# pityka/lamp

Hardware: AMD Instinct MI355X
Metric: training-step samples/sec (higher is better)
Workload: dtype bf16; 1 GPU; example-cifar100 Cnn.resnet(100) training step (fwd+backprop+AdamW), synthetic CIFAR batch; per_gpu_batch=2048, global_batch=2048, parallelism=single, optimizer=AdamW lr 1e-3 wd 0 beta2 0.95 mixedPrecision

## Files before the change

### lamp_amd/csrc/core/switches.h

```cpp
#pragma once
#include <cstdint>

namespace lamp {

constexpr int64_t SW_NO_CLAMP = INT64_MIN;

#define LAMP_SWITCHES_ONCE(X)                                                                                                             \
                                                        \
  X(conv_sibling, "LAMP_CONV_SIBLING", BOOL, 1, 0, "a residual block's 3x3 and its sibling 1x1 of the same input as one forward launch") \
  X(conv_chain, "LAMP_CONV_CHAIN", BOOL, 1, 0, "a convolution directly in front of a residual block and the block's 3x3 + 1x1 as one forward call (0: two)") \
  X(fuse_bn_pair, "LAMP_FUSE_BN_PAIR", BOOL, 1, 0, "relu(bn(right) + bn(left)) at a block's end as one op (0: the chain)")                \
  X(fuse_pool_logsoftmax, "LAMP_FUSE_POOL_LOGSOFTMAX", BOOL, 1, 0, "average pool -> flatten -> log-softmax tail as one node")             \
  X(fuse_block_tail, "LAMP_FUSE_BLOCK_TAIL", BOOL, 1, 0, "the last residual block and the pooled log-softmax tail as one node")          \
  X(fuse_bn_conv, "LAMP_FUSE_BN_CONV", BOOL, 1, 0, "batch norm -> relu -> convolution: the convolution applies the norm while staging")  \
  X(fuse_loss_accumulate, "LAMP_FUSE_LOSS_ACCUMULATE", BOOL, 1, 0, "acc += n * loss inside the NLL loss kernel")                          \
  X(fuse_loss_backward, "LAMP_FUSE_LOSS_BACKWARD", BOOL, 1, 0, "the NLL loss backward goes straight to the pooled log-softmax node's input in one launch")                      \
  X(fuse_loss_tail, "LAMP_FUSE_LOSS_TAIL", BOOL, 1, 0, "the loss launch also writes the pooled log-softmax's input gradient per plane")  \
  X(conv_dgrad_accumulate, "LAMP_CONV_DGRAD_ACCUMULATE", BOOL, 1, 0, "a convolution's input gradient adds into the existing one in its epilogue") \
  X(conv_dgrad_pair, "LAMP_CONV_DGRAD_PAIR", BOOL, 1, 0, "input gradients of a block's 3x3 and sibling 1x1 from one launch")             \
  X(conv_wgrad_pair, "LAMP_CONV_WGRAD_PAIR", BOOL, 1, 0, "weight gradients of a block's 3x3 and sibling 1x1 from one launch")            \
  X(conv_bwd_pair, "LAMP_CONV_BWD_PAIR", BOOL, 1, 0, "a block's paired input gradient and its two weight gradients from one call (0: the two pair calls)") \
  X(linear_bias_fused, "LAMP_LINEAR_BIAS_FUSED", BOOL, 1, 0, "a linear layer's bias in the GEMM epilogue (0: mm then add)")               \
  X(mult_add_fused, "LAMP_MULT_ADD_FUSED", BOOL, 1, 0, "x * scale + residual in one pass (0: mult then add)")                             \
  X(attention_as_written_for_cuda, "LAMP_ATTENTION_AS_WRITTEN_FOR_CUDA", BOOL, 0, 0, "multi-head attention as the reference's op chain instead of the fused kernels") \
  X(recurrent_fused, "LAMP_RECURRENT_FUSED", BOOL, 1, 0, "RNN / GRU / LSTM as one node per sequence with fused cell kernels (0: the fold over time steps)") \
  X(fuse_qkv, "LAMP_FUSE_QKV", BOOL, 1, 0, "self-attention's three projections as one product (0: three)")                                \
  X(host_stream_side, "LAMP_HOST_STREAM_SIDE", BOOL, 0, 0, "batch streams gather on a side stream instead of the consumer's")             \
                                                                           \
  X(pinned_cache_mb, "LAMP_PINNED_CACHE_MB", INT, 2048, 0, "upper bound of the cache of freed pinned host buffers, MiB")                  \
  X(pinned_gather_wgs, "LAMP_PINNED_GATHER_WGS", INT, 48, 1, "workgroups of a gather that reads pinned host memory")                      \
                                                                                                    \
  X(flash_attention, "LAMP_FLASH_ATTENTION", BOOL, 1, 0, "the flash attention kernels, forward and backward")                             \
  X(small_attention, "LAMP_SMALL_ATTENTION", BOOL, 1, 0, "the short-sequence attention kernels")                                          \
  X(knn_fused, "LAMP_KNN_FUSED", BOOL, 1, 0, "the fused distance + top-k nearest-neighbour kernel")                                       \
  X(knn_split, "LAMP_KNN_SPLIT", INT, -1, SW_NO_CLAMP, "f16-plane k-NN filter: 0 off, 1 where it pays, 2 forced; negative: the mode set through the API") \
  X(knn_split_planes, "LAMP_KNN_SPLIT_PLANES", INT, 0, SW_NO_CLAMP, "f16 planes per coordinate of that filter: 3, anything else 2")      \
  X(umap_pairs2, "LAMP_UMAP_PAIRS2", BOOL, 1, 0, "the UMAP loss's two-dimensional pair kernel")                                            \
                                                                                                             \
  X(gemm_shape_tags, "LAMP_GEMM_SHAPE_TAGS", BOOL, 0, 0, "profiling aid: one kernel-timer class per GEMM shape and layout")               \
  X(gemm_splitk, "LAMP_GEMM_SPLITK", BOOL, 1, 0, "split-K for products with few output tiles (bf16 and f32 / f64)")                       \
  X(gemm_tail_split, "LAMP_GEMM_TAIL_SPLIT", BOOL, 1, 0, "an almost empty last round of 256 x 256 tiles becomes a second, split-K product") \
  X(gemm_fp_split_wgs, "LAMP_GEMM_FP_SPLIT_WGS", INT, 512, 1, "workgroups an f32 / f64 split-K product aims at")                          \
                                                                                              \
  X(bn_fused_bwd, "LAMP_BN_FUSED_BWD", BOOL, 1, 0, "one-pass batch-norm backward (workgroups exchange their sums) where no mode is set through the API") \
  X(bn_fused_fp, "LAMP_BN_FUSED_FP", BOOL, 1, 0, "... its f32 / f64 form")                                                               \
  X(bn_fused_np_mask, "LAMP_BN_FUSED_NP_MASK", INT, 24, SW_NO_CLAMP, "bit mask of packets per thread (1 .. 16) at which the one-pass form runs") \
  X(bn_fused_per_cu, "LAMP_BN_FUSED_PER_CU", INT, 1, 1, "workgroups per CU the one-pass form aims at first")                              \
  X(bn_fused_small_bytes, "LAMP_BN_FUSED_SMALL_BYTES", INT, (4 << 20) + 1, SW_NO_CLAMP, "bf16 activations below this many bytes take the one-pass form whatever the mask") \
                          \
  X(conv_small2, "LAMP_CONV_SMALL2", BOOL, 1, 0, "the small-map direct convolution kernels (second generation)")                          \
  X(conv_small2_wgrad, "LAMP_CONV_SMALL2_WGRAD", BOOL, 1, 0, "... their weight gradient")                                                 \
  X(igemm_f32, "LAMP_IGEMM_F32", BOOL, 1, 0, "implicit-GEMM convolution for f32")                                                          \
  X(igemm_f64, "LAMP_IGEMM_F64", BOOL, 1, 0, "implicit-GEMM convolution for f64")                                                          \
  X(conv_bn_stats, "LAMP_CONV_BN_STATS", BOOL, 1, 0, "forward convolutions hand per-image batch-norm statistics of their output on")     \
  X(ncv_bn_stats, "LAMP_NCV_BN_STATS", BOOL, 1, 0, "... the narrow kernels' alone (needs LAMP_CONV_BN_STATS on as well)")                 \
  X(ncv_dgrad_parity, "LAMP_NCV_DGRAD_PARITY", BOOL, 1, 0, "narrow stride-2 pair input gradient: super-tiles by row parity (0: the plain form)") \
  X(pack_cache, "LAMP_PACK_CACHE", BOOL, 1, 0, "packed filter images are cached per parameter and storage version (all four packing backends: core/pack_cache.h)") \
  X(pack_after_step, "LAMP_PACK_AFTER_STEP", BOOL, 1, 0, "the optimiser repacks every cached filter image of all four backends in place (0: lazily at first use)") \
                                                    \
  X(ig_small_d, "LAMP_IG_SMALL_D", BOOL, 1, 0, "the eight-image kernel for at most 64 output channels too")                               \
  X(ig_w8, "LAMP_IG_W8", BOOL, 1, 0, "two-image 128-row kernel: eight waves per image pair at one workgroup per CU or fewer (0: four)")  \
  X(ig_one_image, "LAMP_IG_ONE_IMAGE", BOOL, 1, 0, "... one image per workgroup at one image per CU or fewer (0: pairs)")                 \
  X(ig_bwd_pair, "LAMP_IG_BWD_PAIR", BOOL, 1, 0, "a wide block's short-K entry pair: input gradient and both weight gradients from one eight-image launch (0: the two pair calls)") \
  X(ig_fwd_pair, "LAMP_IG_FWD_PAIR", BOOL, 1, 0, "a wide block's short-K entry pair, forward: the barrier-free eight-image kernel with both filters resident in LDS (0: the eight-image kernel's sibling form)") \
                                                                                                 \
  X(wgrad_group, "LAMP_WGRAD_GROUP", BOOL, 1, 0, "two layers' eight-wave weight gradients parked and launched as one (0: every layer at once)") \
  X(wgrad_min_ips, "LAMP_WGRAD_MIN_IPS", INT, 0, 2, "fewest images per weight-gradient workgroup; unset (0): 2 up to 512 images, 8 above") \
  X(wg8h_dma, "LAMP_WG8H_DMA", BOOL, 1, 0, "eight-wave weight-gradient kernel: dY tiles by LDS-DMA (0: through registers, the bitwise reference of the DMA's hand-counted waits)") \
  X(defer_wgrad_reduce, "LAMP_DEFER_WGRAD_REDUCE", BOOL, 1, 0, "weight-gradient partial sums are reduced in batches, deferred until someone reads them")

#define LAMP_SWITCHES_PER_CALL(X)                                                                                                         \
  X(ig_variant, "LAMP_IG_VARIANT", LETTER, 0, 0, "bf16 implicit GEMM kernel form: b two-image 128-row, d eight-image at any batch; unset or any other letter: by geometry") \
  X(ig_ktail, "LAMP_IG_KTAIL", BOOL, 1, 0, "a 3x3's 1 .. 8 channels beyond the last whole K chunk from their own packed image (0: the padded chunk)") \
  X(knn_split_dbg, "LAMP_KNN_SPLIT_DBG", INT, 0, SW_NO_CLAMP, "3: the k-NN filter's kernel counts visits, candidates and selection cycles per wave and prints them")

using SwType_BOOL = bool;
using SwType_INT = int64_t;
using SwType_LETTER = char;
#define LAMP_SWITCH_MEMBER(member, name, kind, dflt, lo, doc) SwType_##kind member;
struct Switches { LAMP_SWITCHES_ONCE(LAMP_SWITCH_MEMBER) };
struct SwitchesNow { LAMP_SWITCHES_PER_CALL(LAMP_SWITCH_MEMBER) };
#undef LAMP_SWITCH_MEMBER

const Switches& sw();
SwitchesNow sw_now();

}
```

### lamp_amd/csrc/kernels/norm.hip

```cpp
#include "device_utils.h"
#include <atomic>
#include <map>
#include <mutex>
#include <type_traits>
#include "../core/strided.h"
#include "../core/switches.h"

namespace lamp {

template <class A> struct Welford {
  A n, mean, m2;
};
template <class A> __device__ __forceinline__ void wf_add(Welford<A>& w, A x) {
  w.n += A(1);
  A d = x - w.mean;
  w.mean += d / w.n;
  w.m2 += d * (x - w.mean);
}
template <class A> __device__ __forceinline__ Welford<A> wf_merge(const Welford<A>& a, const Welford<A>& b) {
  Welford<A> r;
  r.n = a.n + b.n;
  if (r.n == A(0)) { r.mean = 0; r.m2 = 0; return r; }
  A d = b.mean - a.mean;
  A f = b.n / r.n;
// ... 102 lines not shown
  if (c >= C) return;
  mean[c] = running_mean ? running_mean[c] : store_as<T>(A(0));
  const A v = running_var ? load_as<A>(running_var[c]) : A(1);
  invstd[c] = store_as<T>((A)(A(1) / (A)sqrt((double)(v + (A)eps))));
}
template <class A> __device__ __forceinline__ A bn_affine(A x, A mu, A scale, A bb);
template <> __device__ __forceinline__ float bn_affine<float>(float x, float mu, float scale, float bb) { return __builtin_fmaf(x - mu, scale, bb); }
template <> __device__ __forceinline__ double bn_affine<double>(double x, double mu, double scale, double bb) { return __builtin_fma(x - mu, scale, bb); }
template <class T>
__global__ __launch_bounds__(256) void bn_apply_kernel(const T* __restrict__ x, T* __restrict__ y, const T* __restrict__ mean,
                                                       const T* __restrict__ invstd, const T* __restrict__ w, const T* __restrict__ b,
                                                       int64_t total, int64_t C, int64_t HW, int vec, int relu) {
  using A = acc_t<T>;
  constexpr int W = 16 / sizeof(T);
  if (vec) {
    const int64_t vpp = HW / W, nv = total / W;
    for (int64_t i = blockIdx.x * (int64_t)blockDim.x + threadIdx.x; i < nv; i += (int64_t)gridDim.x * blockDim.x) {
      const int64_t c = (i / vpp) % C;
      const A scale = load_as<A>(invstd[c]) * (w ? load_as<A>(w[c]) : A(1));
      const A mu = load_as<A>(mean[c]);
      const A bb = b ? load_as<A>(b[c]) : A(0);
      Vec<T, W> pk = *reinterpret_cast<const Vec<T, W>*>(x + i * W);
#pragma unroll
      for (int k = 0; k < W; k++) {
        T v = store_as<T>(bn_affine<A>(load_as<A>(pk.v[k]), mu, scale, bb));
        if (relu && load_as<A>(v) < A(0)) v = store_as<T>(A(0));
        pk.v[k] = v;
      }
      *reinterpret_cast<Vec<T, W>*>(y + i * W) = pk;
    }
    return;
  }
  for (int64_t i = blockIdx.x * (int64_t)blockDim.x + threadIdx.x; i < total; i += (int64_t)gridDim.x * blockDim.x) {
    const int64_t c = (i / HW) % C;
    const A scale = load_as<A>(invstd[c]) * (w ? load_as<A>(w[c]) : A(1));
    const A bb = b ? load_as<A>(b[c]) : A(0);
    T v = store_as<T>(bn_affine<A>(load_as<A>(x[i]), load_as<A>(mean[c]), scale, bb));
    if (relu && load_as<A>(v) < A(0)) v = store_as<T>(A(0));
    y[i] = v;
  }
}

template <class T>
__device__ __forceinline__ void bn_merge_channel(const acc_t<T>* __restrict__ partial, int nsplit, int64_t c, int64_t C, int slice, T* __restrict__ save_mean,
                                                 T* __restrict__ save_invstd, T* running_mean, T* running_var, double momentum, double eps,
                                                 acc_t<T>* stat, acc_t<T> (*wpart)[3]) {
  using A = acc_t<T>;
  const int np = nsplit < 0 ? -nsplit : nsplit;
  if (nsplit < 0) {
    const A* pc = partial + (int64_t)c * np * 3;
    const A shift = pc[1];
    A s1 = 0, s2 = 0, sm = 0;
    for (int s = threadIdx.x; s < np; s += blockDim.x) { const A d = pc[s * 3 + 1] - shift; s1 += d; s2 += d * d; sm += pc[s * 3 + 2]; }
    s1 = wave_sum(s1); s2 = wave_sum(s2); sm = wave_sum(sm);
    if ((threadIdx.x & 63) == 0) { wpart[threadIdx.x >> 6][0] = s1; wpart[threadIdx.x >> 6][1] = s2; wpart[threadIdx.x >> 6][2] = sm; }
    __syncthreads();
  }
  if (threadIdx.x < 64) {
    const int lane = threadIdx.x;
    Welford<A> r{0, 0, 0};
    if (nsplit < 0) {
      A s1 = 0, s2 = 0, sm = 0;
      for (int k = 0; k < (int)(blockDim.x >> 6); k++) { s1 += wpart[k][0]; s2 += wpart[k][1]; sm += wpart[k][2]; }
      const A n0 = partial[(int64_t)c * np * 3], shift = partial[(int64_t)c * np * 3 + 1];
      r.n = n0 * (A)np;
      r.mean = shift + s1 / (A)np;
      r.m2 = sm + n0 * (s2 - s1 * s1 / (A)np);
    } else {
      for (int s = lane; s < np; s += 64) {
        const A* p = partial + ((int64_t)s * C + c) * 3;
        r = wf_merge(r, Welford<A>{p[0], p[1], p[2]});
      }
      r = wf_wave(r);
    }
    if (lane == 0) {
      const A var_biased = r.m2 / r.n;
      const A invstd = A(1) / (A)sqrt((double)(var_biased + (A)eps));
      const T m_t = store_as<T>(r.mean), is_t = store_as<T>(invstd);
      stat[0] = load_as<A>(m_t);
      stat[1] = load_as<A>(is_t);
      if (slice == 0) {
        save_mean[c] = m_t;
        save_invstd[c] = is_t;
        if (running_mean) running_mean[c] = store_as<T>((A)((A)momentum * r.mean + (A)(1 - momentum) * load_as<A>(running_mean[c])));
        if (running_var) {
          const A unbiased = r.m2 / (r.n - A(1));
          running_var[c] = store_as<T>((A)((A)momentum * unbiased + (A)(1 - momentum) * load_as<A>(running_var[c])));
        }
      }
    }
  }
  __syncthreads();
}
template <class T>
__global__ __launch_bounds__(256) void bn_affine_table_kernel(const acc_t<T>* __restrict__ partial, int nsplit, T* __restrict__ save_mean, T* __restrict__ save_invstd,
                                                              T* running_mean, T* running_var, double momentum, double eps, const T* __restrict__ w,
                                                              const T* __restrict__ b, int64_t C, float4* __restrict__ affine) {
  using A = acc_t<T>;
  __shared__ A stat[2];
  __shared__ A wpart[4][3];
  const int64_t c = blockIdx.x;
  bn_merge_channel<T>(partial, nsplit, c, C, 0, save_mean, save_invstd, running_mean, running_var, momentum, eps, stat, wpart);
  if (threadIdx.x == 0) affine[c] = make_float4((float)stat[0], (float)(stat[1] * (w ? load_as<A>(w[c]) : A(1))), b ? (float)load_as<A>(b[c]) : 0.f, 0.f);
}
template <class T>
__global__ __launch_bounds__(256) void bn_affine_from_saved_kernel(const T* __restrict__ mean, const T* __restrict__ invstd, const T* __restrict__ w,
                                                                   const T* __restrict__ b, int64_t C, float4* __restrict__ affine) {
  using A = acc_t<T>;
  const int64_t c = blockIdx.x * (int64_t)blockDim.x + threadIdx.x;
  if (c < C) affine[c] = make_float4((float)load_as<A>(mean[c]), (float)(load_as<A>(invstd[c]) * (w ? load_as<A>(w[c]) : A(1))), b ? (float)load_as<A>(b[c]) : 0.f, 0.f);
}
template <class T> struct BnSecond {
  const T* x; const acc_t<T>* partial; int nsplit; T* save_mean; T* save_invstd; T* running_mean; T* running_var; double momentum, eps; const T* w; const T* b;
};

template <class T>
__global__ __launch_bounds__(256) void bn_apply2_kernel(const T* __restrict__ x, T* __restrict__ y, const acc_t<T>* __restrict__ partial, int nsplit,
                                                        T* __restrict__ save_mean, T* __restrict__ save_invstd, T* running_mean, T* running_var,
                                                        double momentum, double eps, const T* __restrict__ w, const T* __restrict__ b, int64_t N,
                                                        int64_t C, int64_t HW, int nblk, int vec, int relu, const T* __restrict__ addend,
                                                        BnSecond<T> second, T* __restrict__ pooled = nullptr) {
  using A = acc_t<T>;
  constexpr int W = 16 / sizeof(T);
  __shared__ A stat[2], stat2[2];
  __shared__ A wpart[4][3];
  const int64_t c = blockIdx.x;
  const int slice = blockIdx.y;
  bn_merge_channel<T>(partial, nsplit, c, C, slice, save_mean, save_invstd, running_mean, running_var, momentum, eps, stat, wpart);
  if (second.x)
    bn_merge_channel<T>(second.partial, second.nsplit, c, C, slice, second.save_mean, second.save_invstd, second.running_mean, second.running_var,
                        second.momentum, second.eps, stat2, wpart);
  const A mu = stat[0];
  const A scale = stat[1] * (w ? load_as<A>(w[c]) : A(1));
  const A bb = b ? load_as<A>(b[c]) : A(0);
  const A mu2 = second.x ? stat2[0] : A(0);
  const A scale2 = second.x ? stat2[1] * (second.w ? load_as<A>(second.w[c]) : A(1)) : A(0);
  const A bb2 = (second.x && second.b) ? load_as<A>(second.b[c]) : A(0);
  const T* __restrict__ adsrc = second.x ? second.x : addend;
  if (vec) {
    const int64_t vpp = HW / W, total = N * vpp;
    for (int64_t i = (int64_t)slice * blockDim.x + threadIdx.x; i < total; i += (int64_t)nblk * blockDim.x) {
      const int64_t n = i / vpp, v = i - n * vpp;
      const int64_t base = (n * C + c) * HW + v * W;
      Vec<T, W> pk, ad;
      { const uint4 t = nt_load16(reinterpret_cast<const uint4*>(x + base)); pk = *reinterpret_cast<const Vec<T, W>*>(&t); }
      if (adsrc) { const uint4 t = nt_load16(reinterpret_cast<const uint4*>(adsrc + base)); ad = *reinterpret_cast<const Vec<T, W>*>(&t); }
#pragma unroll
      for (int k = 0; k < W; k++) {
        T o = store_as<T>(bn_affine<A>(load_as<A>(pk.v[k]), mu, scale, bb));
        if (adsrc) {
          T a = ad.v[k];
          if (second.x) a = store_as<T>(bn_affine<A>(load_as<A>(a), mu2, scale2, bb2));
          o = store_as<T>((A)(load_as<A>(o) + load_as<A>(a)));
        }
        if (relu && load_as<A>(o) < A(0)) o = store_as<T>(A(0));
        pk.v[k] = o;
      }
      if (pooled) {
        A sum = 0;
#pragma unroll
        for (int k = 0; k < W; k++) sum += load_as<A>(pk.v[k]);
        for (int off = (int)vpp >> 1; off > 0; off >>= 1) sum += __shfl_xor(sum, off, 64);
        if (v == 0) pooled[n * C + c] = store_as<T>((A)(sum / (A)HW));
      } else *reinterpret_cast<Vec<T, W>*>(y + base) = pk;
    }
  } else {
    const int64_t total = N * HW;
    for (int64_t i = (int64_t)slice * blockDim.x + threadIdx.x; i < total; i += (int64_t)nblk * blockDim.x) {
      const int64_t n = i / HW, v = i - n * HW;
      const int64_t base = (n * C + c) * HW + v;
      T o = store_as<T>(bn_affine<A>(load_as<A>(x[base]), mu, scale, bb));
      if (adsrc) {
        T a = adsrc[base];
        if (second.x) a = store_as<T>(bn_affine<A>(load_as<A>(a), mu2, scale2, bb2));
        o = store_as<T>((A)(load_as<A>(o) + load_as<A>(a)));
      }
      if (relu && load_as<A>(o) < A(0)) o = store_as<T>(A(0));
      y[base] = o;
    }
  }
}

template <class T>
__global__ __launch_bounds__(256) void bn_bwd_reduce_kernel(const T* __restrict__ dy, const T* __restrict__ x, const T* __restrict__ mean,
                                                            acc_t<T>* __restrict__ partial, int64_t N, int64_t C, int64_t HW, int nsplit, int vec,
                                                            int relu, const T* __restrict__ invstd, const T* __restrict__ w, const T* __restrict__ b,
                                                            const T* __restrict__ addend) {
  using A = acc_t<T>;
  constexpr int W = 16 / sizeof(T);
  __shared__ A sm[2][4];
  const int64_t c = blockIdx.x;
  const int split = blockIdx.y;
  const A mu = load_as<A>(mean[c]);
  const A scale = relu ? load_as<A>(invstd[c]) * (w ? load_as<A>(w[c]) : A(1)) : A(0);
  const A bb = (relu && b) ? load_as<A>(b[c]) : A(0);
  A s1 = 0, s2 = 0;
  if (vec) {
    const int64_t vpp = HW / W, total = N * vpp;
    for (int64_t i = (int64_t)split * blockDim.x + threadIdx.x; i < total; i += (int64_t)nsplit * blockDim.x) {
      const int64_t n = i / vpp, v = i - n * vpp;
      const int64_t base = (n * C + c) * HW + v * W;
      const Vec<T, W> g = *reinterpret_cast<const Vec<T, W>*>(dy + base);
      const Vec<T, W> xv = *reinterpret_cast<const Vec<T, W>*>(x + base);
      Vec<T, W> ad;
      if (addend) ad = *reinterpret_cast<const Vec<T, W>*>(addend + base);
#pragma unroll
      for (int k = 0; k < W; k++) {
        A gg = load_as<A>(g.v[k]);
        const A xx = load_as<A>(xv.v[k]);
        if (relu) {
          T pre = store_as<T>(bn_affine<A>(xx, mu, scale, bb));
          if (addend) pre = store_as<T>((A)(load_as<A>(pre) + load_as<A>(ad.v[k])));
          if (load_as<A>(pre) < A(0)) gg = A(0);
        }
        s1 += gg; s2 += gg * (xx - mu);
      }
    }
  } else {
    const int64_t total = N * HW;
    for (int64_t i = (int64_t)split * blockDim.x + threadIdx.x; i < total; i += (int64_t)nsplit * blockDim.x) {
      const int64_t n = i / HW, v = i - n * HW;
      const int64_t base = (n * C + c) * HW + v;
      A gg = load_as<A>(dy[base]);
      const A xx = load_as<A>(x[base]);
      if (relu) {
        T pre = store_as<T>(bn_affine<A>(xx, mu, scale, bb));
        if (addend) pre = store_as<T>((A)(load_as<A>(pre) + load_as<A>(addend[base])));
        if (load_as<A>(pre) < A(0)) gg = A(0);
      }
      s1 += gg; s2 += gg * (xx - mu);
    }
  }
  s1 = wave_sum(s1); s2 = wave_sum(s2);
  const int lane = threadIdx.x & 63, wid = threadIdx.x >> 6;
  if (lane == 0) { sm[0][wid] = s1; sm[1][wid] = s2; }
  __syncthreads();
  if (threadIdx.x == 0) {
    A a = 0, bsum = 0;
    for (int k = 0; k < (int)(blockDim.x >> 6); k++) { a += sm[0][k]; bsum += sm[1][k]; }
    partial[((int64_t)split * C + c) * 2] = a;
    partial[((int64_t)split * C + c) * 2 + 1] = bsum;
  }
}
template <class T>
__global__ __launch_bounds__(256) void bn_bwd_reduce_col_kernel(const T* __restrict__ dy, const T* __restrict__ x, const T* __restrict__ mean,
                                                                acc_t<T>* __restrict__ partial, int64_t N, int64_t C, int64_t HW, int nsplit) {
  using A = acc_t<T>;
  const int64_t c = blockIdx.x * (int64_t)blockDim.x + threadIdx.x;
  if (c >= C) return;
  const int split = blockIdx.y;
  const A mu = load_as<A>(mean[c]);
  A s1 = 0, s2 = 0;
  for (int64_t n = split; n < N; n += nsplit) {
    const int64_t base = (n * C + c) * HW;
    for (int64_t i = 0; i < HW; i++) {
      const A g = load_as<A>(dy[base + i]);
      s1 += g;
      s2 += g * (load_as<A>(x[base + i]) - mu);
    }
  }
  partial[((int64_t)split * C + c) * 2] = s1;
// ... 679 lines not shown
#undef BN_FUSED_K
}
struct BnPlaneGrad { const bf16_t* p = nullptr; int sn = 0, sc = 0; };
template <class T>
static bool bn_bwd_fused_launch(const Tensor* gc, const Tensor* xc, const Tensor* mean_t, const Tensor* invstd_t, const Tensor* weight, const Tensor* bias,
                                Tensor* dw, Tensor* db, Tensor* dx, Tensor* dadd, const Tensor* addc, const BnGeom& g, int relu, hipStream_t st,
                                const BnDualHost* dualh = nullptr, BnPlaneGrad gplanes = BnPlaneGrad()) {
  constexpr bool BF16 = std::is_same<T, bf16_t>::value;
  constexpr int W = 16 / (int)sizeof(T);
  if (!bn_fused_gate(xc->device(), !BF16) || g.HW % W != 0) return false;
  const int64_t packets = g.N * (g.HW / W);
  if (packets <= 0 || packets >= (int64_t)1 << 30 || xc->numel() / W >= (int64_t)1 << 31) return false;
  if (addc && !relu) return false;
  const bool planes = gplanes.p != nullptr;
  if (planes && !(dualh && g.HW == 64 && gplanes.sn == 1 && g.N % 8 == 0 && gplanes.sc % 8 == 0 && ((uintptr_t)gplanes.p & 15) == 0)) return false;
  const int cus = num_cus();
  const int np_mask = (int)sw().bn_fused_np_mask;
  auto resident = [&](const void* k) { return std::min<int64_t>(BN_FUSED_SLOTS, (int64_t)cus * std::max(1, kernel_occupancy(k, 512, 0))); };
  const void* kfn = nullptr;
  int64_t S = 0, chunk = g.C;
  if constexpr (BF16) {
    if (g.C > BN_FUSED_MAXC) return false;
    const bool any_size = dualh || xc->numel() * 2 < sw().bn_fused_small_bytes;
    for (int wgs = (int)sw().bn_fused_per_cu; wgs >= 1 && !kfn; wgs--) {
      const BnFusedSlices sl = bn_fused_slices(packets, g.C, cus, wgs);
      if (!any_size && !(np_mask & sl.NP)) continue;
      const void* k = bn_fused_kernel_for<T>(sl.NP, relu, addc, dualh, planes);
      if (g.C * sl.s <= resident(k)) { kfn = k; S = sl.s; }
    }
    if (!kfn) return false;
  } else {
    const BnFusedSlices sl = bn_fused_slices(packets, g.C, cus, 1);
    if (!(np_mask & sl.NP)) return false;
    kfn = bn_fused_kernel_for<T>(sl.NP, relu, addc, false, false);
    const int64_t r = resident(kfn);
    if (sl.s > r) return false;
    S = sl.s;
    chunk = std::min<int64_t>(std::min<int64_t>(g.C, r / S), BN_FUSED_MAXC);
  }
  BnFusedSync sync = bn_fused_sync_state(xc->device(), st);
  if (!sync.depart) return false;
  const double passes = (dx ? 3.0 : 2.0) + (addc ? 1.0 : 0.0) + (dadd ? 1.0 : 0.0) - (planes ? 1.0 : 0.0);
  KernelTimer kt("bn_bwd_fused", 0, passes * (double)xc->numel() * sizeof(T), st);
  auto in = [](const Tensor* t) { return t ? t->ptr<T>() : (const T*)nullptr; };
  auto out = [](Tensor* t) { return t ? t->ptr<T>() : (T*)nullptr; };
  const T* dyp = in(gc); const T* xp = in(xc); const T* mp = in(mean_t); const T* ip = in(invstd_t); const T* wp = in(weight); const T* bp = in(bias);
  const T* adp = in(addc);
  T* dwp = out(dw); T* dbp = out(db); T* dxp = out(dx); T* dap = out(dadd);
  BnFusedDual<T> dual{};
  int a_sc = 0;
  if constexpr (BF16) {
    if (planes) { dyp = gplanes.p; a_sc = gplanes.sc; }
    if (dualh) dual = BnFusedDual<T>{in(dualh->mean2), in(dualh->invstd2), in(dualh->w2), in(dualh->b2), out(dualh->dw2), out(dualh->db2)};
  }
  int64_t a_N = g.N; int a_C = (int)g.C, a_HW = (int)g.HW, a_S = (int)S;
  double inv_m = 1.0 / (double)(g.N * g.HW);
  int a_vshift = bn_fused_vshift(g.HW / W);
  int* awp = device_assert_word(xc->device());
  for (int64_t c0 = 0; c0 < g.C; c0 += chunk) {
    int a_c0 = (int)c0;
    const int64_t nc = std::min<int64_t>(chunk, g.C - c0);
    void* args[] = {(void*)&dyp, (void*)&xp, (void*)&mp, (void*)&ip, (void*)&wp, (void*)&bp, (void*)&sync.slots, (void*)&sync.slots2, (void*)&sync.depart, (void*)&dwp,
                    (void*)&dbp, (void*)&dxp, (void*)&a_N, (void*)&a_C, (void*)&a_HW, (void*)&a_S, (void*)&inv_m, (void*)&adp, (void*)&dap, (void*)&a_vshift, (void*)&awp,
                    (void*)&a_c0, (void*)&dual, (void*)&a_sc};
    HIP_CHECK(hipLaunchKernel(kfn, dim3((unsigned)(nc * S)), dim3(512), args, 0, st));
  }
  return true;
}
static BnPlaneGrad plane_broadcast_base(const Tensor* g) {
  BnPlaneGrad r;
  if (!g || g->dtype != kBF16 || g->ndim != 4 || !g->is_device()) return r;
  if (g->sizes[2] * g->sizes[3] <= 1 || g->strides[2] != 0 || g->strides[3] != 0) return r;
  const int64_t sn = g->sizes[0] > 1 ? g->strides[0] : 0, sc = g->sizes[1] > 1 ? g->strides[1] : 0;
  if (sn < 0 || sc < 0 || sn >= ((int64_t)1 << 24) || sc >= ((int64_t)1 << 24) || (g->sizes[0] - 1) * sn + (g->sizes[1] - 1) * sc >= ((int64_t)1 << 31)) return r;
  r.p = g->ptr<bf16_t>(); r.sn = (int)sn; r.sc = (int)sc;
  return r;
}
static void check_cvec(const Tensor* t, int64_t C, int dtype, const char* what) {
  if (!t) return;
  check_device_tensor(t, what);
  LAMP_CHECK(t->numel() == C && t->dtype == dtype && t->is_contiguous(), what << " must be a contiguous [" << C << "] tensor of the input dtype, got " << t->describe());
}

}

using namespace lamp;

extern "C" {

int lamp_bn_backward_mode(int mode) {
  LAMP_API_BEGIN
  LAMP_CHECK(mode >= -1 && mode <= 2, "lamp_bn_backward_mode: mode must be -1, 0, 1 or 2");
  g_bn_bwd_mode.store(mode, std::memory_order_relaxed);
  LAMP_API_END
}

struct BnSecondArgs {
  const lamp_tensor* x; const lamp_tensor* weight; const lamp_tensor* bias; lamp_tensor* running_mean; lamp_tensor* running_var; double momentum, eps;
  lamp_tensor* save_mean = nullptr; lamp_tensor* save_invstd = nullptr;
};
static int bn_forward_impl(lamp_tensor* out3[3], const lamp_tensor* x, const lamp_tensor* weight, const lamp_tensor* bias,
                           lamp_tensor* running_mean, lamp_tensor* running_var, int training, double momentum, double eps, int relu,
                           const lamp_tensor* addend = nullptr, BnSecondArgs* second = nullptr, bool table_only = false, bool* pooled = nullptr) {
  LAMP_API_BEGIN
  check_device_tensor(x, "input");
  BnGeom g = bn_geom(x);
  const bool want_pooled = pooled && *pooled;
  if (pooled) *pooled = false;
  LAMP_CHECK(!table_only || (training && !addend && !second && x->dtype != kF64), "the batch norm table exists in training mode, as an f32 table for f32 / f16 / bf16 inputs");
  Hold addc, x2c, mean2, invstd2;
  if (second) {
    check_device_tensor(second->x, "second input");
    LAMP_CHECK(!addend && relu && training && g.HW >= 64, "the two-batch-norm residual tail exists in training mode for maps of at least 64 elements");
    LAMP_CHECK(second->x->shape() == x->shape() && second->x->dtype == x->dtype, "second input " << second->x->describe() << " does not match input " << x->describe());
    check_cvec(second->weight, g.C, x->dtype, "second weight"); check_cvec(second->bias, g.C, x->dtype, "second bias");
    check_cvec(second->running_mean, g.C, x->dtype, "second running_mean"); check_cvec(second->running_var, g.C, x->dtype, "second running_var");
    x2c = Hold(contiguous(second->x));
    int64_t cs2[1] = {g.C};
    mean2 = Hold(new_tensor(cs2, 1, x->dtype, x->device())); invstd2 = Hold(new_tensor(cs2, 1, x->dtype, x->device()));
  }
  if (addend) {
    check_device_tensor(addend, "addend");
    LAMP_CHECK(relu && training && g.HW >= 64, "the fused batch-norm-add-relu exists in training mode for maps of at least 64 elements");
    LAMP_CHECK(addend->shape() == x->shape() && addend->dtype == x->dtype, "addend " << addend->describe() << " does not match input " << x->describe());
    addc = Hold(contiguous(addend));
  }
  check_cvec(weight, g.C, x->dtype, "weight"); check_cvec(bias, g.C, x->dtype, "bias");
  check_cvec(running_mean, g.C, x->dtype, "running_mean"); check_cvec(running_var, g.C, x->dtype, "running_var");
  Hold xc(contiguous(x));
  int64_t cs[1] = {g.C}, ts[2] = {g.C, 4};
  Hold y(table_only ? new_tensor(ts, 2, kF32, x->device()) : new_like(xc.get()));
  Hold pooled_t;
  Hold mean(new_tensor(cs, 1, x->dtype, x->device())), invstd(new_tensor(cs, 1, x->dtype, x->device()));
  hipStream_t st = current_stream(x->device());
  const int64_t total = x->numel();
  LAMP_DISPATCH_FLOAT(x->dtype, T, {
    using A = acc_t<T>;
    const int vec = (g.HW % (16 / sizeof(T)) == 0) && (((uintptr_t)xc->raw() | (uintptr_t)y->raw() | (uintptr_t)(x2c.get() ? x2c->raw() : nullptr)) & 15) == 0;
    float4* table = table_only ? reinterpret_cast<float4*>(y->raw()) : nullptr;
    if (training) {
      LAMP_CHECK(g.N * g.HW > 0, "batch norm over an empty batch");
      const bool col = g.HW < 64;
      const int64_t blocks = col ? (g.C + 255) / 256 : g.C;
      const int nsplit = pick_split(blocks, g.N);
      int npart = nsplit;
      Hold partial;
      if (!col && std::is_same<A, float>::value) partial = Hold(conv_stats_lookup(xc.get(), g.C, &npart));
      const bool have_stats = partial.get() != nullptr;
      if (!have_stats) {
        npart = nsplit;
        int64_t ps[1] = {(int64_t)nsplit * g.C * 3};
        partial = Hold(new_tensor(ps, 1, acc_dtype<A>(), x->device()));
      }
      T* rm = running_mean ? running_mean->ptr<T>() : (T*)nullptr;
      T* rv = running_var ? running_var->ptr<T>() : (T*)nullptr;
      const T* wp = weight ? weight->ptr<T>() : (const T*)nullptr;
      const T* bp = bias ? bias->ptr<T>() : (const T*)nullptr;
      if (!have_stats) {
        KernelTimer kt("bn_fwd_stats", 0, (double)total * sizeof(T), st);
        if (col) hipLaunchKernelGGL((bn_stats_col_kernel<T>), dim3((unsigned)blocks, nsplit), dim3(256), 0, st, static_cast<const Tensor*>(xc.get())->ptr<T>(), partial->ptr<A>(), g.N, g.C, g.HW, nsplit);
        else hipLaunchKernelGGL((bn_stats_kernel<T>), dim3((unsigned)g.C, nsplit), dim3(256), 0, st, static_cast<const Tensor*>(xc.get())->ptr<T>(), partial->ptr<A>(), g.N, g.C, g.HW, nsplit, vec);
        LAMP_LAUNCH_CHECK();
      }
      BnSecond<T> sec{};
      Hold partial2;
      if (second) {
        LAMP_CHECK(!col && total > 0, "the two-batch-norm residual tail needs maps of at least 64 elements");
        int npart2 = nsplit;
        if (std::is_same<A, float>::value) partial2 = Hold(conv_stats_lookup(x2c.get(), g.C, &npart2));
        const bool have2 = partial2.get() != nullptr;
        if (!have2) {
          npart2 = nsplit;
          int64_t ps[1] = {(int64_t)nsplit * g.C * 3};
          partial2 = Hold(new_tensor(ps, 1, acc_dtype<A>(), x->device()));
          KernelTimer kt("bn_fwd_stats", 0, (double)total * sizeof(T), st);
          hipLaunchKernelGGL((bn_stats_kernel<T>), dim3((unsigned)g.C, nsplit), dim3(256), 0, st, static_cast<const Tensor*>(x2c.get())->ptr<T>(), partial2->ptr<A>(), g.N, g.C, g.HW, nsplit, vec);
          LAMP_LAUNCH_CHECK();
        }
        sec.x = static_cast<const Tensor*>(x2c.get())->ptr<T>();
        sec.partial = static_cast<const Tensor*>(partial2.get())->ptr<A>(); sec.nsplit = have2 ? -npart2 : npart2;
        sec.save_mean = mean2->ptr<T>(); sec.save_invstd = invstd2->ptr<T>();
        sec.running_mean = second->running_mean ? second->running_mean->ptr<T>() : (T*)nullptr;
        sec.running_var = second->running_var ? second->running_var->ptr<T>() : (T*)nullptr;
        sec.momentum = second->momentum; sec.eps = second->eps;
        sec.w = second->weight ? second->weight->ptr<T>() : (const T*)nullptr; sec.b = second->bias ? second->bias->ptr<T>() : (const T*)nullptr;
      }
      if (table_only && !col) {
        hipLaunchKernelGGL((bn_affine_table_kernel<T>), dim3((unsigned)g.C), dim3(256), 0, st, static_cast<const Tensor*>(partial.get())->ptr<A>(),
                           have_stats ? -npart : npart, mean->ptr<T>(), invstd->ptr<T>(), rm, rv, momentum, eps, wp, bp, g.C, table);
        LAMP_LAUNCH_CHECK();
      } else if (!col && total > 0) {
        const int vec2 = (vec && (!addc.get() || ((uintptr_t)addc->data() & 15) == 0)) ? 1 : 0;
        const int64_t vpp = g.HW / (int64_t)(16 / sizeof(T));
        T* poolp = nullptr;
        if (want_pooled && second && vec2 && vpp >= 1 && vpp <= 64 && (vpp & (vpp - 1)) == 0) {
          int64_t ps[2] = {g.N, g.C};
          pooled_t = Hold(new_tensor(ps, 2, x->dtype, x->device()));
          poolp = pooled_t->ptr<T>();
          *pooled = true;
        }
        KernelTimer kt("bn_fwd_apply", 0, ((second ? 3.0 : addc.get() ? 3.0 : 2.0) - (poolp ? 1.0 : 0.0)) * (double)total * sizeof(T), st);
        hipLaunchKernelGGL((bn_apply2_kernel<T>), dim3((unsigned)g.C, nsplit), dim3(256), 0, st, static_cast<const Tensor*>(xc.get())->ptr<T>(), y->ptr<T>(),
                           static_cast<const Tensor*>(partial.get())->ptr<A>(), have_stats ? -npart : npart,
                           mean->ptr<T>(), invstd->ptr<T>(), rm, rv, momentum, eps, wp, bp, g.N, g.C, g.HW, nsplit,
                           vec2, relu, addc.get() ? addc->ptr<T>() : (const T*)nullptr, sec, poolp);
        LAMP_LAUNCH_CHECK();
      } else {
        hipLaunchKernelGGL((bn_finalize_kernel<T>), dim3((unsigned)((g.C * 64 + 255) / 256)), dim3(256), 0, st, partial->ptr<A>(), g.C, nsplit,
                           mean->ptr<T>(), invstd->ptr<T>(), rm, rv, momentum, eps);
        LAMP_LAUNCH_CHECK();
        if (table_only) {
          hipLaunchKernelGGL((bn_affine_from_saved_kernel<T>), dim3((unsigned)((g.C + 255) / 256)), dim3(256), 0, st, mean->ptr<T>(), invstd->ptr<T>(), wp, bp, g.C, table);
          LAMP_LAUNCH_CHECK();
        } else if (total > 0) {
          KernelTimer kt("bn_fwd_apply", 0, 2.0 * (double)total * sizeof(T), st);
          hipLaunchKernelGGL((bn_apply_kernel<T>), dim3(grid_for(total, 256)), dim3(256), 0, st, xc->ptr<T>(), y->ptr<T>(), mean->ptr<T>(), invstd->ptr<T>(),
                             wp, bp, total, g.C, g.HW, vec, relu);
          LAMP_LAUNCH_CHECK();
        }
      }
    } else {
      hipLaunchKernelGGL((bn_eval_stats_kernel<T>), dim3((unsigned)((g.C + 255) / 256)), dim3(256), 0, st,
                         running_mean ? running_mean->ptr<T>() : (const T*)nullptr, running_var ? running_var->ptr<T>() : (const T*)nullptr,
                         mean->ptr<T>(), invstd->ptr<T>(), g.C, eps);
      LAMP_LAUNCH_CHECK();
      if (total > 0) {
        KernelTimer kt("bn_fwd_apply", 0, 2.0 * (double)total * sizeof(T), st);
        hipLaunchKernelGGL((bn_apply_kernel<T>), dim3(grid_for(total, 256)), dim3(256), 0, st, xc->ptr<T>(), y->ptr<T>(), mean->ptr<T>(),
                           invstd->ptr<T>(), weight ? weight->ptr<T>() : (const T*)nullptr, bias ? bias->ptr<T>() : (const T*)nullptr, total,
                           g.C, g.HW, vec, relu);
        LAMP_LAUNCH_CHECK();
      }
    }
  });
  if (!training) {
  }
  out3[0] = pooled_t.get() ? pooled_t.take() : y.take(); out3[1] = mean.take(); out3[2] = invstd.take();
  if (second) { second->save_mean = mean2.take(); second->save_invstd = invstd2.take(); }
  LAMP_API_END
}
int lamp_native_batch_norm(lamp_tensor* out3[3], const lamp_tensor* x, const lamp_tensor* weight, const lamp_tensor* bias,
                           lamp_tensor* running_mean, lamp_tensor* running_var, int training, double momentum, double eps) {
  return bn_forward_impl(out3, x, weight, bias, running_mean, running_var, training, momentum, eps, 0);
}
int lamp_native_batch_norm_relu(lamp_tensor* out3[3], const lamp_tensor* x, const lamp_tensor* weight, const lamp_tensor* bias,
                                lamp_tensor* running_mean, lamp_tensor* running_var, int training, double momentum, double eps) {
  return bn_forward_impl(out3, x, weight, bias, running_mean, running_var, training, momentum, eps, 1);
}

int lamp_batch_norm_affine(lamp_tensor* out3[3], const lamp_tensor* x, const lamp_tensor* weight, const lamp_tensor* bias, lamp_tensor* running_mean,
                           lamp_tensor* running_var, double momentum, double eps) {
  return bn_forward_impl(out3, x, weight, bias, running_mean, running_var, 1, momentum, eps, 1, nullptr, nullptr, true);
}

static int bn_backward_impl(lamp_tensor* out3[3], const lamp_tensor* grad_out, const lamp_tensor* x, const lamp_tensor* weight,
                            const lamp_tensor* bias, const lamp_tensor* running_mean, const lamp_tensor* running_var,
                            const lamp_tensor* save_mean, const lamp_tensor* save_invstd, int training, double eps, const uint8_t mask[3],
                            int relu, const lamp_tensor* addend = nullptr, lamp_tensor** daddend_out = nullptr) {
  LAMP_API_BEGIN
  check_device_tensor(x, "input"); check_device_tensor(grad_out, "grad_out");
  LAMP_CHECK(grad_out->shape() == x->shape() && grad_out->dtype == x->dtype, "grad_out " << grad_out->describe() << " does not match input " << x->describe());
  BnGeom g = bn_geom(x);
  check_cvec(weight, g.C, x->dtype, "weight");
  if (relu) {
    check_cvec(bias, g.C, x->dtype, "bias");
    LAMP_CHECK(g.HW >= 64, "the fused batch-norm-relu backward exists for maps of at least 64 elements, got " << x->describe());
  }
  Hold xc(contiguous(x)), gc(contiguous(grad_out));
  Hold addc, dadd;
  if (addend) {
    check_device_tensor(addend, "addend");
    LAMP_CHECK(relu && training, "the fused batch-norm-add-relu backward exists in training mode");
    LAMP_CHECK(addend->shape() == x->shape() && addend->dtype == x->dtype, "addend " << addend->describe() << " does not match input " << x->describe());
    addc = Hold(contiguous(addend));
    if (daddend_out) dadd = Hold(new_like(xc.get()));
  }
  hipStream_t st = current_stream(x->device());
  int64_t cs[1] = {g.C};
  Hold mean_h, invstd_h;
  const Tensor* mean_t = save_mean;
  const Tensor* invstd_t = save_invstd;
  if (training) {
    LAMP_CHECK(save_mean && save_invstd, "training-mode batch norm backward needs save_mean and save_invstd");
    check_cvec(save_mean, g.C, x->dtype, "save_mean"); check_cvec(save_invstd, g.C, x->dtype, "save_invstd");
  } else {
    check_cvec(running_mean, g.C, x->dtype, "running_mean"); check_cvec(running_var, g.C, x->dtype, "running_var");
    mean_h = Hold(new_tensor(cs, 1, x->dtype, x->device()));
    invstd_h = Hold(new_tensor(cs, 1, x->dtype, x->device()));
// ... 297 lines not shown
```

Measured before the change: 2.328 million samples/s.

## Add register-resident batch-norm forward kernel with overlapped stat merge

Adds a training-mode batch-norm forward kernel that loads each thread's x (and addend or second input) packets into registers up front with non-temporal loads. It overlaps those loads with the per-channel statistics merge and then applies the affine, residual, relu and optional pooling from registers. The point is to touch memory only once per element and hide the finalize latency, instead of re-reading input as bn_apply2_kernel does. A host-side planner picks slices per channel and packets per thread from the CU count. The new path is on by default for bf16 and falls back to the old kernel for unsupported shapes or f16. The cost is heavier register use and many kernel template variants.

```diff
diff --git a/lamp_amd/csrc/core/switches.h b/lamp_amd/csrc/core/switches.h
--- a/lamp_amd/csrc/core/switches.h
+++ b/lamp_amd/csrc/core/switches.h
@@ -71,6 +71,8 @@
 
 #define LAMP_SWITCHES_PER_CALL(X)                                                                                                         \
   X(ig_variant, "LAMP_IG_VARIANT", LETTER, 0, 0, "bf16 implicit GEMM kernel form: b two-image 128-row, d eight-image at any batch; unset or any other letter: by geometry") \
+  X(bn_fwd_reg, "LAMP_BN_FWD_REG", BOOL, 1, 0, "training-mode forward batch norm, vector path: the register kernel with one memory round trip (0: bn_apply2_kernel, its bitwise reference)") \
+  X(bn_fwd_reg_max_slices, "LAMP_BN_FWD_REG_MAX_SLICES", INT, 0, 0, "... at most this many slices per channel, never fewer than four packets per thread need (0: by plan; 1: the fewest - tests reach the many-packet forms on small tensors)") \
   X(ig_ktail, "LAMP_IG_KTAIL", BOOL, 1, 0, "a 3x3's 1 .. 8 channels beyond the last whole K chunk from their own packed image (0: the padded chunk)") \
   X(knn_split_dbg, "LAMP_KNN_SPLIT_DBG", INT, 0, SW_NO_CLAMP, "3: the k-NN filter's kernel counts visits, candidates and selection cycles per wave and prints them")
 
diff --git a/lamp_amd/csrc/kernels/norm.hip b/lamp_amd/csrc/kernels/norm.hip
--- a/lamp_amd/csrc/kernels/norm.hip
+++ b/lamp_amd/csrc/kernels/norm.hip
@@ -208,15 +208,109 @@
       if (slice == 0) {
         save_mean[c] = m_t;
         save_invstd[c] = is_t;
-        if (running_mean) running_mean[c] = store_as<T>((A)((A)momentum * r.mean + (A)(1 - momentum) * load_as<A>(running_mean[c])));
+        if (running_mean) running_mean[c] = store_as<T>(bn_affine<A>((A)momentum, A(0), r.mean, (A)(1 - momentum) * load_as<A>(running_mean[c])));
         if (running_var) {
           const A unbiased = r.m2 / (r.n - A(1));
-          running_var[c] = store_as<T>((A)((A)momentum * unbiased + (A)(1 - momentum) * load_as<A>(running_var[c])));
+          running_var[c] = store_as<T>(bn_affine<A>((A)momentum, A(0), unbiased, (A)(1 - momentum) * load_as<A>(running_var[c])));
         }
       }
     }
   }
   __syncthreads();
+}
+constexpr int BN_MERGE_K = 4;
+constexpr int BN_MERGE_KS = 2;
+template <class A> struct BnMergeReq { A n0, shift, rm, rv, n[BN_MERGE_KS], a[BN_MERGE_K], b[BN_MERGE_K]; };
+template <class T>
+__device__ __forceinline__ BnMergeReq<acc_t<T>> bn_merge_request(const acc_t<T>* __restrict__ partial, int nsplit, int64_t c, int64_t C, const T* running_mean,
+                                                                  const T* running_var, int fin_wave) {
+  using A = acc_t<T>;
+  const int np = nsplit < 0 ? -nsplit : nsplit;
+  const int tid = threadIdx.x;
+  BnMergeReq<A> q;
+  q.n0 = 0; q.shift = 0;
+#pragma unroll
+  for (int k = 0; k < BN_MERGE_KS; k++) q.n[k] = 0;
+#pragma unroll
+  for (int k = 0; k < BN_MERGE_K; k++) { q.a[k] = 0; q.b[k] = 0; }
+  if (nsplit < 0) {
+    const A* pc = partial + (int64_t)c * np * 3;
+    q.n0 = pc[0]; q.shift = pc[1];
+#pragma unroll
+    for (int k = 0; k < BN_MERGE_K; k++) {
+      const int s = tid + k * 256, ss = s < np ? s : 0;
+      q.a[k] = pc[ss * 3 + 1]; q.b[k] = pc[ss * 3 + 2];
+    }
+  } else {
+    const int lane = tid & 63;
+    const bool mine = (tid >> 6) == fin_wave;
+#pragma unroll
+    for (int k = 0; k < BN_MERGE_KS; k++) {
+      const int s = lane + k * 64, ss = (mine && s < np) ? s : 0;
+      const A* p = partial + ((int64_t)ss * C + c) * 3;
+      q.n[k] = p[0]; q.a[k] = p[1]; q.b[k] = p[2];
+    }
+  }
+  q.rm = running_mean ? load_as<A>(running_mean[c]) : A(0);
+  q.rv = running_var ? load_as<A>(running_var[c]) : A(0);
+  return q;
+}
+template <class T>
+__device__ __forceinline__ void bn_merge_reduce(const BnMergeReq<acc_t<T>>& q, const acc_t<T>* __restrict__ partial, int nsplit, int64_t c, acc_t<T> (*wpart)[3]) {
+  using A = acc_t<T>;
+  if (nsplit >= 0) return;
+  const int np = -nsplit, tid = threadIdx.x;
+  const A* pc = partial + (int64_t)c * np * 3;
+  A s1 = 0, s2 = 0, sm = 0;
+#pragma unroll
+  for (int k = 0; k < BN_MERGE_K; k++)
+    if (tid + k * 256 < np) { const A d = q.a[k] - q.shift; s1 += d; s2 += d * d; sm += q.b[k]; }
+  for (int s = tid + BN_MERGE_K * 256; s < np; s += 256) { const A d = pc[s * 3 + 1] - q.shift; s1 += d; s2 += d * d; sm += pc[s * 3 + 2]; }
+  s1 = wave_sum(s1); s2 = wave_sum(s2); sm = wave_sum(sm);
+  if ((tid & 63) == 0) { wpart[tid >> 6][0] = s1; wpart[tid >> 6][1] = s2; wpart[tid >> 6][2] = sm; }
+}
+template <class T>
+__device__ __forceinline__ void bn_merge_finalise(const BnMergeReq<acc_t<T>>& q, const acc_t<T>* __restrict__ partial, int nsplit, int64_t c, int64_t C, int slice,
+                                                  T* __restrict__ save_mean, T* __restrict__ save_invstd, T* running_mean, T* running_var, double momentum,
+                                                  double eps, acc_t<T>* stat, acc_t<T> (*wpart)[3], int fin_wave) {
+  using A = acc_t<T>;
+  const int np = nsplit < 0 ? -nsplit : nsplit;
+  if ((int)(threadIdx.x >> 6) != fin_wave) return;
+  const int lane = threadIdx.x & 63;
+  Welford<A> r{0, 0, 0};
+  if (nsplit < 0) {
+    A s1 = 0, s2 = 0, sm = 0;
+    for (int k = 0; k < 4; k++) { s1 += wpart[k][0]; s2 += wpart[k][1]; sm += wpart[k][2]; }
+    const A n0 = q.n0, shift = q.shift;
+    r.n = n0 * (A)np;
+    r.mean = shift + s1 / (A)np;
+    r.m2 = sm + n0 * (s2 - s1 * s1 / (A)np);
+  } else {
+#pragma unroll
+    for (int k = 0; k < BN_MERGE_KS; k++)
+      if (lane + k * 64 < np) r = wf_merge(r, Welford<A>{q.n[k], q.a[k], q.b[k]});
+    for (int s = lane + BN_MERGE_KS * 64; s < np; s += 64) {
+      const A* p = partial + ((int64_t)s * C + c) * 3;
+      r = wf_merge(r, Welford<A>{p[0], p[1], p[2]});
+    }
+    r = wf_wave(r);
+  }
+  if (lane == 0) {
+    const A var_biased = r.m2 / r.n;
+    const A invstd = A(1) / (A)sqrt((double)(var_biased + (A)eps));
+    const T m_t = store_as<T>(r.mean), is_t = store_as<T>(invstd);
+    stat[0] = load_as<A>(m_t);
+    stat[1] = load_as<A>(is_t);
+    if (slice == 0) {
+      save_mean[c] = m_t;
+      save_invstd[c] = is_t;
+      if (running_mean) running_mean[c] = store_as<T>(bn_affine<A>((A)momentum, A(0), r.mean, (A)(1 - momentum) * q.rm));
+      if (running_var) {
+        const A unbiased = r.m2 / (r.n - A(1));
+        running_var[c] = store_as<T>(bn_affine<A>((A)momentum, A(0), unbiased, (A)(1 - momentum) * q.rv));
+      }
+    }
+  }
 }
 template <class T>
 __global__ __launch_bounds__(256) void bn_affine_table_kernel(const acc_t<T>* __restrict__ partial, int nsplit, T* __restrict__ save_mean, T* __restrict__ save_invstd,
@@ -303,6 +397,98 @@
       }
       if (relu && load_as<A>(o) < A(0)) o = store_as<T>(A(0));
       y[base] = o;
+    }
+  }
+}
+
+template <class T, int NP, int FORM>
+__global__ __launch_bounds__(256) void bn_fwd_reg_kernel(const T* __restrict__ x, T* __restrict__ y, const acc_t<T>* __restrict__ partial, int nsplit,
+                                                         T* __restrict__ save_mean, T* __restrict__ save_invstd, T* running_mean, T* running_var,
+                                                         double momentum, double eps, const T* __restrict__ w, const T* __restrict__ b, int64_t N, int C,
+                                                         int HW, int S, int vshift, int relu, const T* __restrict__ addend, BnSecond<T> second,
+                                                         T* __restrict__ pooled) {
+  using A = acc_t<T>;
+  constexpr int W = 16 / sizeof(T);
+  constexpr bool TWO = FORM >= 1, SECOND = FORM >= 2, POOLED = FORM == 3;
+  __shared__ A stat[2][2];
+  __shared__ A wpart[2][4][3];
+  const int c = blockIdx.x, s = blockIdx.y, tid = threadIdx.x;
+  const unsigned vpp = (unsigned)HW / (unsigned)W;
+  const unsigned total = (unsigned)N * vpp;
+  const BnMergeReq<A> q1 = bn_merge_request<T>(partial, nsplit, c, C, running_mean, running_var, 0);
+  BnMergeReq<A> q2 = q1;
+  if constexpr (SECOND) q2 = bn_merge_request<T>(second.partial, second.nsplit, c, C, second.running_mean, second.running_var, 1);
+  const T* x0 = x + (size_t)c * (unsigned)HW;
+  const T wv = *(w ? w + c : x0), bv = *(b ? b + c : x0);
+  const T wv2 = SECOND ? *(second.w ? second.w + c : x0) : wv, bv2 = SECOND ? *(second.b ? second.b + c : x0) : bv;
+  const uint4* x4 = reinterpret_cast<const uint4*>(x);
+  const uint4* ad4 = reinterpret_cast<const uint4*>(SECOND ? second.x : addend);
+  uint4 xv[NP], av[TWO ? NP : 1];
+#pragma unroll
+  for (int k = 0; k < NP; k++) {
+    const unsigned i = (unsigned)(k * S + s) * 256u + (unsigned)tid;
+    const unsigned ii = i < total ? i : 0u;
+    const unsigned n = vshift >= 0 ? (ii >> vshift) : (ii / vpp);
+    const unsigned idx = (n * (unsigned)C + (unsigned)c) * vpp + (ii - n * vpp);
+    xv[k] = nt_load16(x4 + idx);
+    if constexpr (TWO) av[k] = nt_load16(ad4 + idx);
+  }
+  bn_merge_reduce<T>(q1, partial, nsplit, c, wpart[0]);
+  if constexpr (SECOND) bn_merge_reduce<T>(q2, second.partial, second.nsplit, c, wpart[1]);
+  __syncthreads();
+  bn_merge_finalise<T>(q1, partial, nsplit, c, C, s, save_mean, save_invstd, running_mean, running_var, momentum, eps, stat[0], wpart[0], 0);
+  if constexpr (SECOND)
+    bn_merge_finalise<T>(q2, second.partial, second.nsplit, c, C, s, second.save_mean, second.save_invstd, second.running_mean, second.running_var,
+                         second.momentum, second.eps, stat[1], wpart[1], 1);
+  __syncthreads();
+  const A mu = stat[0][0];
+  const A scale = stat[0][1] * (w ? load_as<A>(wv) : A(1));
+  const A bb = b ? load_as<A>(bv) : A(0);
+  const A mu2 = SECOND ? stat[1][0] : A(0);
+  const A scale2 = SECOND ? stat[1][1] * (second.w ? load_as<A>(wv2) : A(1)) : A(0);
+  const A bb2 = (SECOND && second.b) ? load_as<A>(bv2) : A(0);
+  unsigned tid2 = (unsigned)tid;
+  asm volatile("" : "+v"(tid2));
+  A psum[POOLED ? NP : 1];
+#pragma unroll
+  for (int k = 0; k < NP; k++) {
+    const unsigned i = (unsigned)(k * S + s) * 256u + tid2;
+    const bool valid = i < total;
+    const unsigned ii = valid ? i : 0u;
+    const unsigned n = vshift >= 0 ? (ii >> vshift) : (ii / vpp);
+    const unsigned v = ii - n * vpp;
+    const unsigned idx = (n * (unsigned)C + (unsigned)c) * vpp + v;
+    Vec<T, W> pk = *reinterpret_cast<const Vec<T, W>*>(&xv[k]);
+    const Vec<T, W> ad = *reinterpret_cast<const Vec<T, W>*>(&av[TWO ? k : 0]);
+#pragma unroll
+    for (int j = 0; j < W; j++) {
+      T o = store_as<T>(bn_affine<A>(load_as<A>(pk.v[j]), mu, scale, bb));
+      if constexpr (TWO) {
+        T a = ad.v[j];
+        if constexpr (SECOND) a = store_as<T>(bn_affine<A>(load_as<A>(a), mu2, scale2, bb2));
+        o = store_as<T>((A)(load_as<A>(o) + load_as<A>(a)));
+      }
+      if (relu && load_as<A>(o) < A(0)) o = store_as<T>(A(0));
+      pk.v[j] = o;
+    }
+    if constexpr (POOLED) {
+      A sum = 0;
+#pragma unroll
+      for (int j = 0; j < W; j++) sum += load_as<A>(pk.v[j]);
+      psum[k] = sum;
+    } else if (valid) *reinterpret_cast<Vec<T, W>*>(y + (size_t)idx * W) = pk;
+    __builtin_amdgcn_sched_barrier(0);
+  }
+  if constexpr (POOLED) {
+    for (int off = (int)vpp >> 1; off > 0; off >>= 1) {
+#pragma unroll
+      for (int k = 0; k < NP; k++) psum[k] += __shfl_xor(psum[k], off, 64);
+    }
+#pragma unroll
+    for (int k = 0; k < NP; k++) {
+      const unsigned i = (unsigned)(k * S + s) * 256u + tid2;
+      const unsigned n = vshift >= 0 ? (i >> vshift) : (i / vpp);
+      if (i < total && i - n * vpp == 0) pooled[(size_t)n * (unsigned)C + (unsigned)c] = store_as<T>((A)(psum[k] / (A)HW));
     }
   }
 }
@@ -1148,11 +1334,72 @@
   LAMP_CHECK(t->numel() == C && t->dtype == dtype && t->is_contiguous(), what << " must be a contiguous [" << C << "] tensor of the input dtype, got " << t->describe());
 }
 
+
+struct BnFwdPlan { int S = 0, NP = 0; int64_t wgs = 0; int rounds = 0; };
+static int bn_fwd_reg_per_cu(int held) { return held <= 1 ? 8 : 7; }
+static int bn_fwd_reg_np(int64_t packets, int64_t S) {
+  const int64_t ppt = (packets + S * 256 - 1) / (S * 256);
+  return ppt <= 1 ? 1 : ppt <= 2 ? 2 : 4;
+}
+static BnFwdPlan bn_fwd_plan(int64_t N, int64_t C, int64_t HW, int esize, bool two, bool pooled, int cus, int64_t max_slices = 0) {
+  BnFwdPlan p;
+  const int64_t W = 16 / esize;
+  if (N <= 0 || C <= 0 || HW < 64 || HW % W != 0 || cus <= 0) return p;
+  const int64_t vpp = HW / W, packets = N * vpp;
+  if (packets >= (int64_t)1 << 30 || packets * C >= (int64_t)1 << 31) return p;
+  if (pooled && (vpp > 64 || (vpp & (vpp - 1)) != 0)) return p;
+  const int np_max = two ? 2 : 4;
+  const int64_t s_min = (packets + 256 * np_max - 1) / (256 * np_max), s_max = (packets + 255) / 256;
+  int64_t S = 0;
+  if (max_slices > 0) S = std::max(s_min, std::min(s_max, max_slices));
+  for (int np = 1; np <= np_max && !S; np *= 2) {
+    const int64_t lo = (packets + 256 * np - 1) / (256 * np);
+    const int64_t hi = np == 1 ? s_max : (packets + 128 * np - 1) / (128 * np) - 1;
+    const int64_t s = std::min(hi, (int64_t)cus * bn_fwd_reg_per_cu(np * (two ? 2 : 1)) / C);
+    if (s >= lo && bn_fwd_reg_np(packets, s) == np) S = s;
+  }
+  if (!S || S > 65535) return p;
+  p.S = (int)S;
+  p.NP = bn_fwd_reg_np(packets, S);
+  p.wgs = C * S;
+  const int64_t room = (int64_t)cus * bn_fwd_reg_per_cu(p.NP * (two ? 2 : 1));
+  p.rounds = (int)((p.wgs + room - 1) / room);
+  return p;
+}
+template <class T>
+static const void* bn_fwd_reg_kernel_for(int NP, int form) {
+#define BN_FWD_K(NPv, F) ((const void*)bn_fwd_reg_kernel<T, NPv, F>)
+#define BN_FWD_NP2(F) (NP == 1 ? BN_FWD_K(1, F) : BN_FWD_K(2, F))
+  return form == 0 ? (NP == 4 ? BN_FWD_K(4, 0) : BN_FWD_NP2(0)) : form == 1 ? BN_FWD_NP2(1) : form == 2 ? BN_FWD_NP2(2) : BN_FWD_NP2(3);
+#undef BN_FWD_NP2
+#undef BN_FWD_K
+}
+
 }
 
 using namespace lamp;
 
 extern "C" {
+
+int lamp_debug_bn_fwd_plan(int64_t N, int64_t C, int64_t HW, int esize, int two, int pooled, int aligned, int cus, int max_slices, char* buf, int buflen) {
+  LAMP_API_BEGIN
+  LAMP_CHECK(buf && buflen > 0 && cus > 0 && (esize == 2 || esize == 4 || esize == 8), "lamp_debug_bn_fwd_plan: bad arguments");
+  const BnFwdPlan p = aligned ? bn_fwd_plan(N, C, HW, esize, two != 0, pooled != 0, cus, max_slices) : BnFwdPlan();
+  char line[128];
+  if (p.NP) snprintf(line, sizeof(line), "reg S=%d NP=%d wgs=%lld rounds=%d", p.S, p.NP, (long long)p.wgs, p.rounds);
+  else snprintf(line, sizeof(line), "old");
+  LAMP_CHECK((int)strlen(line) < buflen, "lamp_debug_bn_fwd_plan: buffer too small");
+  memcpy(buf, line, strlen(line) + 1);
+  LAMP_API_END
+}
+int lamp_debug_conv_stats_partials(const lamp_tensor* x, int* count) {
+  LAMP_API_BEGIN
+  LAMP_CHECK(x && count && x->ndim >= 2, "lamp_debug_conv_stats_partials: bad arguments");
+  int P = 0;
+  Hold part(conv_stats_lookup(x, x->sizes[1], &P));
+  *count = part.get() ? P : 0;
+  LAMP_API_END
+}
 
 int lamp_bn_backward_mode(int mode) {
   LAMP_API_BEGIN
@@ -1266,10 +1513,28 @@
           *pooled = true;
         }
         KernelTimer kt("bn_fwd_apply", 0, ((second ? 3.0 : addc.get() ? 3.0 : 2.0) - (poolp ? 1.0 : 0.0)) * (double)total * sizeof(T), st);
-        hipLaunchKernelGGL((bn_apply2_kernel<T>), dim3((unsigned)g.C, nsplit), dim3(256), 0, st, static_cast<const Tensor*>(xc.get())->ptr<T>(), y->ptr<T>(),
-                           static_cast<const Tensor*>(partial.get())->ptr<A>(), have_stats ? -npart : npart,
-                           mean->ptr<T>(), invstd->ptr<T>(), rm, rv, momentum, eps, wp, bp, g.N, g.C, g.HW, nsplit,
-                           vec2, relu, addc.get() ? addc->ptr<T>() : (const T*)nullptr, sec, poolp);
+        const T* xp = static_cast<const Tensor*>(xc.get())->ptr<T>();
+        const T* adp = addc.get() ? addc->ptr<T>() : (const T*)nullptr;
+        const A* pp = static_cast<const Tensor*>(partial.get())->ptr<A>();
+        int a_nsplit = have_stats ? -npart : npart;
+        BnFwdPlan plan;
+        if (vec2 && !std::is_same<T, f16_t>::value && sw_now().bn_fwd_reg)
+          plan = bn_fwd_plan(g.N, g.C, g.HW, (int)sizeof(T), second || adp, poolp != nullptr, num_cus(), sw_now().bn_fwd_reg_max_slices);
+        if constexpr (!std::is_same<T, f16_t>::value) {
+          if (plan.NP) {
+            const void* kfn = bn_fwd_reg_kernel_for<T>(plan.NP, second ? (poolp ? 3 : 2) : adp ? 1 : 0);
+            T* yp = y->ptr<T>(); T* mp = mean->ptr<T>(); T* ip = invstd->ptr<T>();
+            int64_t a_N = g.N; int a_C = (int)g.C, a_HW = (int)g.HW, a_S = plan.S, a_vshift = bn_fused_vshift(g.HW / (int64_t)(16 / sizeof(T))), a_relu = relu;
+            double a_mom = momentum, a_eps = eps;
+            void* args[] = {(void*)&xp, (void*)&yp, (void*)&pp, (void*)&a_nsplit, (void*)&mp, (void*)&ip, (void*)&rm, (void*)&rv, (void*)&a_mom, (void*)&a_eps,
+                            (void*)&wp, (void*)&bp, (void*)&a_N, (void*)&a_C, (void*)&a_HW, (void*)&a_S, (void*)&a_vshift, (void*)&a_relu, (void*)&adp, (void*)&sec,
+                            (void*)&poolp};
+            HIP_CHECK(hipLaunchKernel(kfn, dim3((unsigned)g.C, (unsigned)plan.S), dim3(256), args, 0, st));
+          }
+        }
+        if (!plan.NP)
+          hipLaunchKernelGGL((bn_apply2_kernel<T>), dim3((unsigned)g.C, nsplit), dim3(256), 0, st, xp, y->ptr<T>(), pp, a_nsplit,
+                             mean->ptr<T>(), invstd->ptr<T>(), rm, rv, momentum, eps, wp, bp, g.N, g.C, g.HW, nsplit, vec2, relu, adp, sec, poolp);
         LAMP_LAUNCH_CHECK();
       } else {
         hipLaunchKernelGGL((bn_finalize_kernel<T>), dim3((unsigned)((g.C * 64 + 255) / 256)), dim3(256), 0, st, partial->ptr<A>(), g.C, nsplit,
```

Result: no change. 2.339 million samples/s (median of 6 runs) (+0.5%).
